# leerob/pixo

Hardware: NVIDIA H100
Metric: Mpixels/sec JPEG q=80 4:2:0 encode of 3840x2160 RGB (higher is better)
Workload: dtype f32

## Files before the change

### pixo_b200/csrc/api.cu

```cuda
#include <stdarg.h>
#include <stdlib.h>
#include <string.h>

#include <emmintrin.h>

#include <algorithm>
#include <cmath>
#include <thread>
#include <vector>

#include "common.cuh"
#include "jpeg_host.hpp"

namespace pixo {

static thread_local std::string g_thread_err;

int set_error(pixo_b200_ctx *ctx, int code, const char *fmt, ...)
{
    char buf[512];
    va_list ap;
    va_start(ap, fmt);
    vsnprintf(buf, sizeof buf, fmt, ap);
    va_end(ap);
// ... 1026 lines not shown
                                         uint32_t n_frames, uint32_t width, uint32_t height, uint32_t color_type,
                                         uint32_t subsampling, const uint8_t *dht, uint8_t *d_out,
                                         size_t out_cap_each, uint64_t *d_scan_len, uint32_t *d_overflow)
{
    if (!ctx) return set_error(nullptr, PIXO_B200_ERR_INVALID_ARGUMENT, "ctx is null");
    PIXO_TRY(validate_jpeg(ctx, width, height, color_type, subsampling));
    const bool chroma = color_type != PIXO_B200_GRAY;
    if (!d_y || !d_out || !d_scan_len || !d_overflow || (chroma && (!d_cb || !d_cr)))
        return set_error(ctx, PIXO_B200_ERR_INVALID_ARGUMENT, "null buffer");
    const FrameGeometry g = make_geometry(width, height, color_type, subsampling);
    auto mis = [](const int16_t *p) { return (reinterpret_cast<uintptr_t>(p) & 15) != 0; };
    if (mis(d_y) || (chroma && (mis(d_cb) || mis(d_cr))))
        return set_error(ctx, PIXO_B200_ERR_INVALID_ARGUMENT, "coefficient arrays must be 16-byte aligned");
    if ((y_stride & 7) || (chroma && (c_stride & 7)))
        return set_error(ctx, PIXO_B200_ERR_INVALID_ARGUMENT, "coefficient strides must be multiples of 8 elements");
    if (n_frames > 1 && (y_stride < g.ny * 64 || (chroma && c_stride < g.nc * 64)))
        return set_error(ctx, PIXO_B200_ERR_INVALID_ARGUMENT,
                         "coefficient strides must hold a frame's blocks (%zu / %zu elements)", g.ny * 64, g.nc * 64);
    ProgTables T;
    {
        HuffTables std_t;
        uint8_t bits[4][16];
        const uint8_t *vals[4];
        if (dht) {
            for (int k = 0; k < 4; ++k) {
                memcpy(bits[k], dht + k * 272, 16);
                vals[k] = dht + k * 272 + 16;
            }
        } else {
            huff_standard(std_t);
            for (int k = 0; k < 4; ++k) {
                memcpy(bits[k], std_t.bits[k], 16);
                vals[k] = std_t.vals[k];
            }
        }
        if (!prog_tables(bits, vals, &T))
            return set_error(ctx, PIXO_B200_ERR_INVALID_ARGUMENT,
                             "Huffman table: more than 256 values, or a code that does not fit its length");
    }
    if (n_frames == 0) return 0;
    PIXO_CUDA(ctx, cudaSetDevice(ctx->device));
    constexpr uint32_t kPass = 8192;
    const int16_t *cb = chroma ? d_cb : nullptr, *cr = chroma ? d_cr : nullptr;
    auto at = [](const int16_t *a, size_t stride, uint32_t i0) { return a ? a + (size_t)i0 * stride : nullptr; };
    ProgResult res;
    if (n_frames > kPass)
        for (uint32_t i0 = 0; i0 < n_frames; i0 += kPass)
            PIXO_TRY(launch_progressive(ctx, at(d_y, y_stride, i0), y_stride, at(cb, c_stride, i0), at(cr, c_stride, i0),
                                        c_stride, std::min(kPass, n_frames - i0), g, &T, false, true, &res));
    for (uint32_t i0 = 0; i0 < n_frames; i0 += kPass) {
        const uint32_t cnt = std::min(kPass, n_frames - i0);
        PIXO_TRY(launch_progressive(ctx, at(d_y, y_stride, i0), y_stride, at(cb, c_stride, i0), at(cr, c_stride, i0),
                                    c_stride, cnt, g, &T, false, false, &res));
        PIXO_TRY(launch_progressive_pack(ctx, res, cnt, d_out + (size_t)i0 * out_cap_each, out_cap_each,
                                         d_scan_len + (size_t)i0 * 7, d_overflow + i0));
    }
    return 0;
}

int pixo_b200_jpeg_encode_dev(pixo_b200_ctx *ctx, const uint8_t *d_pixels, size_t pixel_stride,
                              uint32_t n_images, uint32_t width, uint32_t height,
                              uint32_t color_type, uint32_t quality, uint32_t subsampling,
                              uint8_t *d_scan, size_t scan_cap_each, uint64_t *d_scan_len,
                              uint32_t *d_overflow)
{
    if (!ctx) return set_error(nullptr, PIXO_B200_ERR_INVALID_ARGUMENT, "ctx is null");
    PIXO_TRY(validate_options(ctx, quality, 0));
    PIXO_TRY(validate_jpeg(ctx, width, height, color_type, subsampling));
    if (!d_pixels || !d_scan || !d_scan_len || !d_overflow)
        return set_error(ctx, PIXO_B200_ERR_INVALID_ARGUMENT, "null buffer");
    if (n_images == 0) return 0;
    if (n_images > 65535) return set_error(ctx, PIXO_B200_ERR_INVALID_ARGUMENT, "at most 65535 frames per call");
    if (scan_cap_each % 4 || (reinterpret_cast<uintptr_t>(d_scan) & 15))
        return set_error(ctx, PIXO_B200_ERR_INVALID_ARGUMENT, "scan buffer must be 16-byte aligned, capacity multiple of 4");
    const FrameGeometry g = make_geometry(width, height, color_type, subsampling);
    float lum[64], chr[64];
    quant_tables((int)quality, nullptr, nullptr, lum, chr);
    const CoefLayout L(g);
    PIXO_CUDA(ctx, cudaSetDevice(ctx->device));
    PIXO_TRY(ensure_dev(ctx, ctx->d_coef, (size_t)n_images * L.each));
    PIXO_TRY(ensure_dev(ctx, ctx->d_ent, entropy_scratch_bytes(n_images, g, 0)));
    void *c = ctx->d_coef.ptr;
    const CoefExtents ec = L.extents(c);
    PIXO_TRY(launch_jpeg_transform(ctx, d_pixels, pixel_stride, n_images, width, height, color_type, subsampling,
                                   lum, chr, L.y(c), L.stride(), g.has_chroma ? L.cb(c) : nullptr,
                                   g.has_chroma ? L.cr(c) : nullptr, L.stride(), 0, &ec));
    HuffTables t;
    huff_standard(t);
    uint64_t *len_src = nullptr;
    uint32_t *ovf_src = nullptr;
    PIXO_TRY(launch_jpeg_entropy(ctx, L.y(c), L.stride(), L.cb(c), L.cr(c), L.stride(), n_images, g, t, 0, true, &ec,
                                 reinterpret_cast<uint8_t *>(ctx->d_ent.ptr), d_scan, scan_cap_each,
                                 &len_src, &ovf_src));
    PIXO_CUDA(ctx, cudaMemcpyAsync(d_scan_len, len_src, (size_t)n_images * 8, cudaMemcpyDeviceToDevice, ctx->stream));
    PIXO_CUDA(ctx, cudaMemcpyAsync(d_overflow, ovf_src, (size_t)n_images * 4, cudaMemcpyDeviceToDevice, ctx->stream));
    return 0;
}

static int check_range(pixo_b200_ctx *ctx, const int16_t *y, const int16_t *cb, const int16_t *cr,
                       const FrameGeometry &g, uint32_t restart_interval, const int32_t *seed)
{
    if (!coefficients_in_range(y, g.ny, restart_interval, g.y_per_mcu, seed ? seed[0] : 0) ||
        (g.has_chroma && (!coefficients_in_range(cb, g.nc, restart_interval, 1, seed ? seed[1] : 0) ||
                          !coefficients_in_range(cr, g.nc, restart_interval, 1, seed ? seed[2] : 0))))
        return set_error(ctx, PIXO_B200_ERR_INVALID_ARGUMENT, "%s", kOutOfRange);
    return 0;
}

static int check_coef_alignment(pixo_b200_ctx *ctx, const int16_t *d_y, const int16_t *d_cb, const int16_t *d_cr,
                                bool has_chroma)
{
    auto mis = [](const int16_t *p) { return (reinterpret_cast<uintptr_t>(p) & 15) != 0; };
    if (mis(d_y) || (has_chroma && (mis(d_cb) || mis(d_cr))))
        return set_error(ctx, PIXO_B200_ERR_INVALID_ARGUMENT, "coefficient arrays must be 16-byte aligned");
    return 0;
}

int pixo_b200_jpeg_entropy_encode(pixo_b200_ctx *ctx, const int16_t *y, const int16_t *cb,
                                  const int16_t *cr, uint32_t width, uint32_t height,
                                  uint32_t color_type, uint32_t quality, uint32_t subsampling,
                                  uint32_t restart_interval, uint32_t optimize_huffman,
                                  uint8_t *out, size_t out_cap, size_t *out_len)
{
    PIXO_TRY(validate_options(ctx, quality, restart_interval));
    PIXO_TRY(validate_jpeg(ctx, width, height, color_type, subsampling));
    if (!y || !out || !out_len || (color_type != PIXO_B200_GRAY && (!cb || !cr)))
        return set_error(ctx, PIXO_B200_ERR_INVALID_ARGUMENT, "null buffer");
    const FrameGeometry g = make_geometry(width, height, color_type, subsampling);
    PIXO_TRY(check_range(ctx, y, cb, cr, g, restart_interval, nullptr));
    if (out_cap < 1024 + 2)
        return set_error(ctx, PIXO_B200_ERR_OUTPUT_TOO_SMALL, "output capacity %zu too small", out_cap);
    uint64_t hist[536];
    if (optimize_huffman) host_histogram(y, cb, cr, g, restart_interval, hist);
    HuffTables t;
    tables_from(optimize_huffman ? hist : nullptr, g.has_chroma, t);
    uint8_t lum_zz[64], chr_zz[64];
    quant_tables((int)quality, lum_zz, chr_zz, nullptr, nullptr);
    const size_t hdr = write_headers(out, g, lum_zz, chr_zz, t, restart_interval);
    int threads = ctx ? ctx->host_threads : (int)std::thread::hardware_concurrency();
    const size_t body = entropy_encode_scan(y, cb, cr, g, t, restart_interval, false, out + hdr, out_cap - hdr - 2,
                                            threads < 1 ? 1 : threads);
    return finish_frame(ctx, out, out_cap, hdr, body, out_len);
}

int pixo_b200_jpeg_entropy_encode_dev(pixo_b200_ctx *ctx, const int16_t *d_y, const int16_t *d_cb,
                                      const int16_t *d_cr, uint32_t width, uint32_t height,
                                      uint32_t color_type, uint32_t quality, uint32_t subsampling,
                                      uint32_t restart_interval, uint32_t optimize_huffman,
                                      uint8_t *out, size_t out_cap, size_t *out_len)
{
    if (!ctx) return set_error(nullptr, PIXO_B200_ERR_INVALID_ARGUMENT, "ctx is null");
    PIXO_TRY(validate_options(ctx, quality, restart_interval));
    PIXO_TRY(validate_jpeg(ctx, width, height, color_type, subsampling));
    if (!d_y || !out || !out_len || (color_type != PIXO_B200_GRAY && (!d_cb || !d_cr)))
        return set_error(ctx, PIXO_B200_ERR_INVALID_ARGUMENT, "null buffer");
    if (out_cap < 1024 + 2)
        return set_error(ctx, PIXO_B200_ERR_OUTPUT_TOO_SMALL, "output capacity %zu too small", out_cap);
    const FrameGeometry g = make_geometry(width, height, color_type, subsampling);
    PIXO_TRY(check_coef_alignment(ctx, d_y, d_cb, d_cr, g.has_chroma));
    uint8_t lum_zz[64], chr_zz[64];
    quant_tables((int)quality, lum_zz, chr_zz, nullptr, nullptr);
    PIXO_CUDA(ctx, cudaSetDevice(ctx->device));
    uint64_t *h_hist = nullptr;
    if (optimize_huffman) {
        PIXO_TRY(ensure_dev(ctx, ctx->d_misc, kHistWords * sizeof(uint64_t) + 256));
        PIXO_TRY(ensure_pinned(ctx, ctx->h_misc, kHistWords * sizeof(uint64_t) + 256));
        auto *d_hist = reinterpret_cast<uint64_t *>(ctx->d_misc.ptr);
        h_hist = reinterpret_cast<uint64_t *>(ctx->h_misc.ptr);
        PIXO_TRY(launch_jpeg_histogram(ctx, d_y, 0, d_cb, d_cr, 0, 1, g.ny, g.nc, g.y_per_mcu, restart_interval,
                                       false, nullptr, d_hist));
        PIXO_CUDA(ctx, cudaMemcpyAsync(h_hist, d_hist, kHistWords * sizeof(uint64_t), cudaMemcpyDeviceToHost, ctx->stream));
        PIXO_CUDA(ctx, cudaStreamSynchronize(ctx->stream));
    }
    HuffTables t;
    tables_from(h_hist, g.has_chroma, t);
    const size_t hdr = write_headers(out, g, lum_zz, chr_zz, t, restart_interval);
    const size_t raw = (size_t)width * height * (color_type == PIXO_B200_GRAY ? 1 : 3);
// ... 458 lines not shown
```

### pixo_b200/csrc/common.cuh

```cuda
#pragma once

#include <cuda_runtime.h>
#include <stdint.h>
#include <stdio.h>

#include <atomic>
#include <condition_variable>
#include <functional>
#include <mutex>
#include <string>
#include <thread>
#include <unordered_map>
#include <vector>

#include "../../include/pixo_b200.h"

namespace pixo {

constexpr int kHistWords = 536;

__host__ __device__ constexpr int zz_nat(int i)
{
    constexpr int t[64] = {0,  1,  8,  16, 9,  2,  3,  10, 17, 24, 32, 25, 18, 11, 4,  5,
                           12, 19, 26, 33, 40, 48, 41, 34, 27, 20, 13, 6,  7,  14, 21, 28,
// ... 63 lines not shown
    size_t stage_cap = 0;
    uint64_t *d_len = nullptr;
    std::vector<uint64_t> len;
};

}

struct pixo_b200_ctx {
    int device = 0;
    cudaStream_t own_stream = nullptr;
    cudaStream_t stream = nullptr;
    cudaStream_t copy_stream = nullptr;
    cudaStream_t d2h_stream = nullptr;
    int sm_count = 0;
    int host_threads = 0;
    uint64_t launches = 0;
    uint64_t host_fallbacks = 0;
    size_t scan_cap_override = 0;
    bool gpu_retry = true;
    std::string err;
    pixo::Scratch d_in, d_y, d_cb, d_cr, d_misc, d_out, d_ent, d_coef, d_retry, d_raw;
    pixo::Scratch d_red, d_red_idx, d_red_img;
    pixo::Scratch d_quant, d_quant_img;
    pixo::Scratch d_trellis, h_trellis;
    pixo::Scratch d_prog, d_prog_raw, d_prog_out, h_prog;
    pixo::Scratch h_in, h_out, h_misc, h_red, h_quant;
    std::vector<cudaEvent_t> events;
    std::vector<cudaEvent_t> stage_events;
    pixo::HostPool *pool = nullptr;
    std::unordered_map<const void *, pixo::SegPlan> bands;
};

namespace pixo {

int set_error(pixo_b200_ctx *ctx, int code, const char *fmt, ...);
int cuda_fail(pixo_b200_ctx *ctx, cudaError_t e, const char *what);
int ensure_dev(pixo_b200_ctx *ctx, Scratch &s, size_t bytes);
int ensure_pinned(pixo_b200_ctx *ctx, Scratch &s, size_t bytes);

#define PIXO_CUDA(ctx, call)                                            \
    do {                                                                \
        cudaError_t e__ = (call);                                       \
        if (e__ != cudaSuccess) return ::pixo::cuda_fail(ctx, e__, #call); \
    } while (0)

#define PIXO_TRY(expr)                 \
    do {                               \
        int rc__ = (expr);             \
        if (rc__ != 0) return rc__;    \
    } while (0)

int launch_jpeg_transform(pixo_b200_ctx *ctx, const uint8_t *d_pixels, size_t pixel_stride,
                          uint32_t n_images, uint32_t w, uint32_t h, uint32_t color_type,
                          uint32_t subsampling, const float *lum_q, const float *chr_q,
                          int16_t *d_y, size_t y_stride, int16_t *d_cb, int16_t *d_cr,
                          size_t c_stride, uint32_t flags, const CoefExtents *ext = nullptr);
int launch_jpeg_transform_dct(pixo_b200_ctx *ctx, const uint8_t *d_pixels, size_t pixel_stride, uint32_t n_images,
                              uint32_t w, uint32_t h, uint32_t color_type, uint32_t subsampling,
                              const float *lum_q, const float *chr_q, float *d_y, size_t y_stride, float *d_cb,
                              float *d_cr, size_t c_stride);
int launch_trellis(pixo_b200_ctx *ctx, const float *d_src, size_t src_stride, int16_t *d_dst, size_t dst_stride,
                   uint64_t nb, uint32_t n_frames, const float q[64], float lambda, bool zigzag, uint32_t *d_status);
int launch_jpeg_histogram(pixo_b200_ctx *ctx, const int16_t *d_y, size_t y_stride,
                          const int16_t *d_cb, const int16_t *d_cr, size_t c_stride,
                          uint32_t n_images, size_t ny, size_t nc, uint32_t blocks_y_per_mcu,
                          uint32_t restart_interval, bool zigzag_in, const CoefExtents *ext, uint64_t *d_hist,
                          const int *dc_seed = nullptr);
int launch_png_filter_rows(pixo_b200_ctx *ctx, const uint8_t *d_data, size_t in_stride, uint32_t n_images,
                           uint32_t width, uint32_t height, size_t row_bytes, uint32_t bpp, uint32_t strategy,
                           uint8_t *d_out, size_t out_stride, uint32_t *d_adler, const uint8_t *d_above,
                           uint32_t rule_height);
int launch_adler32(pixo_b200_ctx *ctx, const uint8_t *d_data, size_t len, uint32_t *d_out);
int png_reduce_filter(pixo_b200_ctx *ctx, const uint8_t *d_data, size_t in_stride, uint32_t n_images,
                      uint32_t width, uint32_t height, uint32_t color_type, uint32_t strategy_and_flags,
                      pixo_b200_png_reduced *info, uint8_t *d_out, size_t out_stride, uint32_t *d_adler);
int png_quantize_filter(pixo_b200_ctx *ctx, const uint8_t *d_data, size_t in_stride, uint32_t n_images,
                        uint32_t width, uint32_t height, uint32_t color_type, uint32_t strategy_and_flags,
                        uint32_t max_colors, const uint8_t *palettes, const uint32_t *palette_lens,
                        pixo_b200_png_reduced *info, uint8_t *d_out, size_t out_stride, uint32_t *d_adler);

struct FrameGeometry;
struct HuffTables;
size_t entropy_scratch_bytes(uint32_t n, const FrameGeometry &g, uint32_t restart_interval);
int launch_jpeg_entropy(pixo_b200_ctx *ctx, const int16_t *d_y, size_t y_stride, const int16_t *d_cb,
                        const int16_t *d_cr, size_t c_stride, uint32_t n, const FrameGeometry &g,
                        const HuffTables &t, uint32_t restart_interval, bool allow_segments,
                        const CoefExtents *ext, uint8_t *d_scratch, uint8_t *d_out, uint64_t out_cap,
                        uint64_t **d_out_len, uint32_t **d_overflow);
int launch_band_entropy(pixo_b200_ctx *ctx, const int16_t *d_y, const int16_t *d_cb, const int16_t *d_cr,
                        const FrameGeometry &g, const HuffTables &t, const int dc_seed[3], const int *d_dc_seed,
                        bool allow_segments, uint8_t *d_raw, uint64_t raw_cap, uint64_t *d_bits_tail,
                        uint32_t *d_flags);
int launch_band_splice(pixo_b200_ctx *ctx, const uint8_t *d_raw, uint64_t base_bit, uint32_t base_tail, bool last,
                       const uint64_t *d_base, uint8_t *d_out, uint64_t out_cap, uint64_t *d_out_len,
                       uint32_t *d_flags);
size_t band_raw_bytes(const FrameGeometry &g);
SegPlan splice_plan(uint32_t n, size_t raw_cap);
int launch_splice(pixo_b200_ctx *ctx, uint32_t n, const SegPlan &sp, uint8_t *seg_scratch, const uint8_t *raw_area,
                  uint8_t *d_out, uint64_t out_cap, uint64_t *d_out_len, uint32_t *d_overflow);

bool prog_tables(const uint8_t bits[4][16], const uint8_t *const vals[4], ProgTables *T);
ProgLayout prog_layout(const FrameGeometry &g, uint32_t n);
int launch_progressive(pixo_b200_ctx *ctx, const int16_t *d_y, size_t y_stride, const int16_t *d_cb,
                       const int16_t *d_cr, size_t c_stride, uint32_t n, const FrameGeometry &g,
                       const ProgTables *T, bool per_frame, bool check_only, ProgResult *res);
int launch_progressive_pack(pixo_b200_ctx *ctx, const ProgResult &res, uint32_t n, uint8_t *d_out, uint64_t out_cap,
                            uint64_t *d_scan_len, uint32_t *d_overflow);

}
```

### pixo_b200/csrc/jpeg_entropy.cu

```cuda
#include "common.cuh"
#include "jpeg_host.hpp"

namespace pixo {
namespace {

constexpr int AC_STRIDE = 12, AC_ZRL = 190, AC_EOB = 191, AC_WORDS = 192;
struct HuffDev {
    uint32_t dc[2][12];
    uint32_t ac[2][AC_WORDS];
};

struct EntParams {
    const int16_t *y, *cb, *cr;
    size_t y_stride, c_stride;
    CoefExtents e;
    uint32_t bpm;
    uint32_t y_per_mcu;
    uint32_t nblocks;
    uint32_t nchunks;
    uint32_t rst_mcus;
    uint32_t rst_blocks;
    uint32_t cpi;
    uint32_t nimages;
    unsigned long long *st_bits;
// ... 185 lines not shown
        while (mb) {
            const uint32_t f = msb_index(mb);
            uint32_t bit;
            asm("bmsk.clamp.b32 %0, %1, 1;" : "=r"(bit) : "r"(f));
            mb ^= bit;
            const uint32_t pos = top - f;
            uint32_t run = pos + nprev;
            nprev = ~pos;
            uint32_t caddr;
            asm("{\n\t.reg .b32 h, x;\n\tand.b32 h, %1, 1;\n\tmad.lo.u32 x, %1, 64, %2;\n\tmad.lo.u32 %0, h, -62, x;\n\t}"
                : "=r"(caddr) : "r"(pos), "r"(sa_stage));
            const int c = lds_s16(caddr);
#pragma unroll 1
            while (run >= 16u) { put(zrl & 0xFFFF0000u, zrl & 31u); run -= 16u; }
            const uint32_t a = (uint32_t)abs(c);
            if (CHECK) amax |= a >> 10;
            const uint32_t lz = CHECK ? max((uint32_t)__clz((int)a), 22u) : (uint32_t)__clz((int)a);
            const uint32_t e = lds_u32(sa_ac_top + run * (AC_STRIDE * 4u) - lz * 4u);
            const uint32_t amp = a ^ ((uint32_t)(c >> 31) >> lz);
            const uint32_t n = e & 31u;
            put((e & 0xFFFF0000u) | __funnelshift_r(0u, amp, n), n);
        }
    }
    if (nprev != ~63u) put(eob & 0xFFFF0000u, eob & 31u);
    *acc_out = acc;
    *bad = amax != 0;
    return ((sp - sa_slot) / (CB * 4)) * 32u + filled;
}

__device__ __forceinline__ uint32_t warp_scan(uint32_t x, int lane, uint32_t *total)
{
    uint32_t inc = x;
#pragma unroll
    for (int o = 1; o < 32; o <<= 1) {
        const uint32_t n = __shfl_up_sync(0xffffffffu, inc, o);
        if (lane >= o) inc += n;
    }
    *total = __shfl_sync(0xffffffffu, inc, 31);
    return inc - x;
}

struct WarpMem {
    uint32_t slot[2][SLOT_W * CB];
    union {
        uint32_t stage[32 * CB];
        struct {
            uint32_t obuf[WIN_W];
            uint8_t sbuf[SBUF_B];
        } w;
    };
    uint32_t tl[CB];
};

struct ChunkState {
    uint32_t chunk, img;
    uint32_t L, o_t;
    int nwt;
    uint32_t Lc, ctail;
    int buf;
    unsigned long long Pc;
    uint32_t tailin;
    uint32_t Ftot;
    uint32_t own;
    uint32_t marker;
    bool first, last, final_;
    uint32_t ffb;
    bool kept;
    bool fault;
    bool skip;
};

template <bool RAW, bool CHECK>
__global__ void __launch_bounds__(32 * HUFF_WARPS, HUFF_CTAS_PER_SM)
k_huff(const __grid_constant__ EntParams P, const __grid_constant__ HuffDev Tp)
{
    __shared__ HuffDev T;
    __shared__ __align__(16) WarpMem wmem[HUFF_WARPS];
    static_assert(sizeof(((WarpMem *)0)->w) <= sizeof(((WarpMem *)0)->stage), "window + stuffed bytes must fit the stage");

    const int lane = threadIdx.x & 31;
    for (int i = threadIdx.x; i < (int)(sizeof(HuffDev) / 4); i += blockDim.x)
        reinterpret_cast<uint32_t *>(&T)[i] = reinterpret_cast<const uint32_t *>(&Tp)[i];
    __syncthreads();
    WarpMem &M = wmem[threadIdx.x >> 5];
    uint32_t *const obuf = M.w.obuf;
    uint8_t *const sbuf = M.w.sbuf;
    const uint32_t sa_stage = (uint32_t)__cvta_generic_to_shared(M.stage) + 4u * lane;
    const uint32_t total_chunks = P.nchunks * P.nimages;
    uint32_t spill[2][MAX_W - SLOT_W];

    auto phase_w = [&](uint32_t id, int buf, ChunkState &C) {
        C.chunk = id / P.nimages;
        C.img = id - C.chunk * P.nimages;
        C.buf = buf;
        C.fault = false;
        uint32_t s0, iend, interval = 0;
        uint32_t nblk = P.nblocks;
        size_t y_off = (size_t)C.img * P.y_stride, c_off = (size_t)C.img * P.c_stride;
        size_t ey_off = (size_t)C.img * P.e.stride, ec_off = ey_off;
        bool seg_prev = false;
        if (RAW && P.seg_per_img > 1) {
            const uint32_t ii = C.img / P.seg_per_img, seg = C.img - ii * P.seg_per_img;
            y_off = (size_t)ii * P.y_stride + (size_t)seg * P.seg_y_stride;
            c_off = (size_t)ii * P.c_stride + (size_t)seg * P.seg_c_stride;
            ey_off = (size_t)ii * P.e.stride + (size_t)seg * (P.seg_y_stride / 64);
            ec_off = (size_t)ii * P.e.stride + (size_t)seg * (P.seg_c_stride / 64);
            if (seg == P.seg_per_img - 1) nblk = P.nblocks_last;
            seg_prev = seg != 0;
        }
        C.skip = false;
        if (P.rst_blocks) {
            interval = C.chunk / P.cpi;
            const uint32_t sub = C.chunk - interval * P.cpi;
            s0 = interval * P.rst_blocks + sub * CB;
            iend = (uint32_t)min((unsigned long long)(interval + 1) * P.rst_blocks, (unsigned long long)nblk);
            C.first = sub == 0;
        } else {
            s0 = C.chunk * CB;
            iend = nblk;
            C.first = C.chunk == 0;
        }
        if (s0 >= iend) { C.skip = true; return; }
        C.last = s0 + CB >= iend;
        C.final_ = C.last && iend == nblk;
        C.marker = (C.last && !C.final_) ? 0xD0u + (interval & 7u) : 0u;
        const uint32_t s = s0 + lane;
        const int nv = (int)min((uint32_t)CB, iend - s0);
        uint32_t *const slot = M.slot[buf];
        uint32_t L = 0, tail7 = 0;
        int nwt = 0;
        uint32_t M0 = 0, M1 = 0;
        int diff = 0, tbl = 0;
        if (s < iend) {
            const uint32_t m = s / P.bpm;
            const uint32_t k = s - m * P.bpm;
            const int16_t *arr;
            const uint8_t *earr;
            size_t idx, eidx;
            int seed;
            if (k < P.y_per_mcu) { arr = P.y + y_off; earr = P.e.y; idx = (size_t)m * P.y_per_mcu + k; eidx = ey_off + idx; tbl = 0; seed = P.dc_seed[0]; }
            else if (k == P.y_per_mcu) { arr = P.cb + c_off; earr = P.e.cb; idx = m; eidx = ec_off + idx; tbl = 1; seed = P.dc_seed[1]; }
            else { arr = P.cr + c_off; earr = P.e.cr; idx = m; eidx = ec_off + idx; tbl = 1; seed = P.dc_seed[2]; }
            const bool dc_reset = P.rst_mcus && m % P.rst_mcus == 0 && (k == 0 || k >= P.y_per_mcu);
            if (P.dc_seed_dev && idx == 0 && !seg_prev) seed = P.dc_seed_dev[k < P.y_per_mcu ? 0 : (k == P.y_per_mcu ? 1 : 2)];
            const int prev_dc = dc_reset ? 0 : ((idx || seg_prev) ? arr[((long long)idx - 1) * 64] : seed);
            const uint4 *src = reinterpret_cast<const uint4 *>(arr + idx * 64);
            int dc;
            uint32_t w[32];
            if (CHECK) {
                uint32_t n[32];
#pragma unroll
                for (int q = 0; q < 8; ++q) {
                    const uint4 v = __ldg(src + q);
                    n[q * 4] = v.x; n[q * 4 + 1] = v.y; n[q * 4 + 2] = v.z; n[q * 4 + 3] = v.w;
                }
                dc = (int)(int16_t)(n[0] & 0xFFFF);
#pragma unroll
                for (int j = 0; j < 32; ++j) {
                    const int i0 = zz_nat(2 * j), i1 = zz_nat(2 * j + 1);
                    w[j] = __byte_perm(n[i0 >> 1], n[i1 >> 1],
                                       ((i0 & 1) ? 0x0032 : 0x0010) | ((i1 & 1) ? 0x7600 : 0x5400));
                }
#pragma unroll
                for (int j = 0; j < 32; ++j) M.stage[j * CB + lane] = w[j];
            } else {
                const int np = 2 * __ldg(earr + eidx);
// ... 714 lines not shown

static SegPlan plan_segments(uint32_t n, uint32_t S, uint64_t total_mcus, uint64_t bpm, uint64_t mcu_raw_bytes)
{
    SegPlan p;
    p.seg_mcus = (total_mcus + S - 1) / S;
    S = (uint32_t)((total_mcus + p.seg_mcus - 1) / p.seg_mcus);
    p.S = S;
    p.last_mcus = total_mcus - p.seg_mcus * (S - 1);
    const uint64_t fair = p.seg_mcus * mcu_raw_bytes + 4096, worst = p.seg_mcus * bpm * 216 + 64;
    lay_out(p, n, bpm, (size_t)a256(std::min(fair, worst)));
    return p;
}

static uint64_t mcu_raw_bytes(const FrameGeometry &g) { return (uint64_t)g.y_per_mcu * 64 * (g.has_chroma ? 3 : 1); }

static int code_segments(pixo_b200_ctx *ctx, EntParams P, const HuffDev &T, uint32_t n, const FrameGeometry &g,
                         const SegPlan &sp, uint8_t *seg_scratch, uint8_t *raw_area)
{
    const bool check = P.e.y == nullptr;
    cudaStream_t st = ctx->stream;
    const uint64_t bpm = g.y_per_mcu + (g.has_chroma ? 2 : 0);
    uint8_t *ent = seg_scratch + sp.off_ent;
    P.nimages = n * sp.S;
    P.seg_per_img = sp.S;
    P.nblocks = (uint32_t)(sp.seg_mcus * bpm);
    P.nblocks_last = (uint32_t)(sp.last_mcus * bpm);
    P.nchunks = (uint32_t)sp.ent.nchunks;
    P.seg_y_stride = (size_t)sp.seg_mcus * g.y_per_mcu * 64;
    P.seg_c_stride = (size_t)sp.seg_mcus * 64;
    P.rst_blocks = P.rst_mcus = P.cpi = 0;
    P.st_bits = reinterpret_cast<unsigned long long *>(ent + sp.ent.off_st1);
    P.st_ff = reinterpret_cast<unsigned long long *>(ent + sp.ent.off_st2);
    P.ticket = reinterpret_cast<uint32_t *>(ent + sp.ent.off_ticket);
    P.overflow = reinterpret_cast<uint32_t *>(ent + sp.ent.off_ovf);
    P.out_len = reinterpret_cast<uint64_t *>(ent + sp.ent.off_outlen);
    P.out_tail = reinterpret_cast<unsigned long long *>(ent + sp.ent.off_tail);
    P.out = raw_area;
    P.out_cap = sp.raw_cap;
    PIXO_CUDA(ctx, cudaMemsetAsync(ent, 0, sp.ent.zero_bytes, st));
    const size_t want = ((size_t)P.nimages * P.nchunks + HUFF_WARPS - 1) / HUFF_WARPS;
    const unsigned grid = (unsigned)std::min<size_t>(want, (size_t)ctx->sm_count * HUFF_CTAS_PER_SM);
    if (check) k_huff<true, true><<<grid, 32 * HUFF_WARPS, 0, st>>>(P, T);
    else k_huff<true, false><<<grid, 32 * HUFF_WARPS, 0, st>>>(P, T);
    ctx->launches += 1;
    PIXO_CUDA(ctx, cudaGetLastError());
    PIXO_CUDA(ctx, cudaMemcpyAsync(raw_area + sp.off_bits, P.out_len, (size_t)n * sp.S * 8, cudaMemcpyDeviceToDevice, st));
    PIXO_CUDA(ctx, cudaMemcpyAsync(raw_area + sp.off_tails, P.out_tail, (size_t)n * sp.S * 8, cudaMemcpyDeviceToDevice, st));
    return 0;
}

static int splice_segments(pixo_b200_ctx *ctx, uint32_t n, const SegPlan &sp, uint8_t *seg_scratch,
                           const uint8_t *raw_area, const uint32_t *raw_overflow, uint64_t base_bit, uint32_t base_tail,
                           bool last, const uint64_t *base_dev, uint8_t *d_out, uint64_t out_cap, uint64_t *d_out_len,
                           uint32_t *d_overflow)
{
    cudaStream_t st = ctx->stream;
    SegParams Q;
    Q.raw = raw_area; Q.raw_cap = sp.raw_cap;
    Q.bits = reinterpret_cast<const unsigned long long *>(raw_area + sp.off_bits);
    Q.tails = reinterpret_cast<const unsigned long long *>(raw_area + sp.off_tails);
    Q.S = sp.S; Q.max_tiles = sp.max_tiles;
    Q.base_bit = base_bit; Q.base_tail = base_tail; Q.last_band = last ? 1u : 0u;
    Q.base_dev = reinterpret_cast<const unsigned long long *>(base_dev);
    Q.rec = reinterpret_cast<SegRec *>(seg_scratch + sp.off_rec);
    Q.ntiles = reinterpret_cast<uint32_t *>(seg_scratch + sp.off_ntiles);
    Q.cnt = reinterpret_cast<uint32_t *>(seg_scratch + sp.off_cnt);
    Q.out = d_out; Q.out_cap = out_cap;
    Q.out_len = reinterpret_cast<unsigned long long *>(d_out_len);
    Q.overflow = d_overflow;
    Q.raw_overflow = raw_overflow;
    k_seg_prefix<<<n, SPL_THREADS, 0, st>>>(Q);
    k_seg_count<<<dim3((sp.max_tiles + SPL_TPC - 1) / SPL_TPC, n), SPL_THREADS, 0, st>>>(Q);
    k_seg_scan<<<n, 1024, 0, st>>>(Q);
    k_seg_emit<<<dim3((sp.max_tiles + SPL_TPC - 1) / SPL_TPC, n), SPL_THREADS, 0, st>>>(Q);
    ctx->launches += 4;
    PIXO_CUDA(ctx, cudaGetLastError());
    return 0;
}

int launch_jpeg_entropy(pixo_b200_ctx *ctx, const int16_t *d_y, size_t y_stride, const int16_t *d_cb,
                        const int16_t *d_cr, size_t c_stride, uint32_t n, const FrameGeometry &g,
                        const HuffTables &t, uint32_t restart_interval, bool allow_segments,
                        const CoefExtents *ext, uint8_t *d_scratch, uint8_t *d_out, uint64_t out_cap,
                        uint64_t **d_out_len, uint32_t **d_overflow)
{
    const bool check = ext == nullptr;
    const uint64_t nblocks = g.ny + 2 * g.nc;
    const uint64_t bpm_ = g.y_per_mcu + (g.has_chroma ? 2 : 0);
    uint64_t rst_blocks = (uint64_t)restart_interval * bpm_;
    if (rst_blocks >= nblocks) rst_blocks = 0;
    const EntropyPlan pl = plan_entropy(n, nblocks, rst_blocks);
    if (nblocks > 0xFFFFFFFFull || (uint64_t)n * pl.nchunks > 0x7FFFFFFFull)
        return set_error(ctx, PIXO_B200_ERR_INVALID_ARGUMENT, "entropy stage: too many blocks per call");
    EntParams P;
    P.y = d_y; P.cb = d_cb; P.cr = d_cr; P.y_stride = y_stride; P.c_stride = c_stride;
    P.e = ext ? *ext : CoefExtents{nullptr, nullptr, nullptr, 0};
    P.bpm = g.y_per_mcu + (g.has_chroma ? 2 : 0);
    P.y_per_mcu = g.y_per_mcu;
    P.nblocks = (uint32_t)nblocks;
    P.nchunks = (uint32_t)pl.nchunks;
    P.rst_blocks = (uint32_t)rst_blocks;
    P.rst_mcus = rst_blocks ? restart_interval : 0u;
    P.cpi = rst_blocks ? (uint32_t)((rst_blocks + CB - 1) / CB) : 0u;
    P.nimages = n;
    P.st_bits = reinterpret_cast<unsigned long long *>(d_scratch + pl.off_st1);
    P.st_ff = reinterpret_cast<unsigned long long *>(d_scratch + pl.off_st2);
    P.ticket = reinterpret_cast<uint32_t *>(d_scratch + pl.off_ticket);
    P.overflow = reinterpret_cast<uint32_t *>(d_scratch + pl.off_ovf);
    P.out_len = reinterpret_cast<uint64_t *>(d_scratch + pl.off_outlen);
    P.out = d_out; P.out_cap = out_cap;
    P.out_tail = reinterpret_cast<unsigned long long *>(d_scratch + pl.off_tail);
    P.dc_seed[0] = P.dc_seed[1] = P.dc_seed[2] = 0;
    P.dc_seed_dev = nullptr;
    *d_out_len = P.out_len;
    *d_overflow = P.overflow;

    HuffDev T;
    make_huff_dev(t, &T);
    cudaStream_t st = ctx->stream;
    PIXO_CUDA(ctx, cudaMemsetAsync(d_scratch, 0, pl.zero_bytes, st));
    P.seg_per_img = 1; P.nblocks_last = P.nblocks; P.seg_y_stride = P.seg_c_stride = 0;
    const uint32_t S = (rst_blocks == 0 && allow_segments) ? segments_for(n, g.total_mcus(), bpm_) : 1;
    const SegPlan sp = plan_segments(n, S, g.total_mcus(), bpm_, mcu_raw_bytes(g));
    if (sp.S > 1) {
        PIXO_TRY(ensure_dev(ctx, ctx->d_raw, sp.total + sp.raw_total));
        auto *seg_scratch = reinterpret_cast<uint8_t *>(ctx->d_raw.ptr);
        uint8_t *raw_area = seg_scratch + sp.total;
        PIXO_TRY(code_segments(ctx, P, T, n, g, sp, seg_scratch, raw_area));
        return splice_segments(ctx, n, sp, seg_scratch, raw_area,
                               reinterpret_cast<const uint32_t *>(seg_scratch + sp.off_ent + sp.ent.off_ovf), 0, 0, true,
                               nullptr, d_out, out_cap, P.out_len, P.overflow);
    }
    const size_t want = ((size_t)n * pl.nchunks + HUFF_WARPS - 1) / HUFF_WARPS;
    const unsigned grid = (unsigned)std::min<size_t>(want, (size_t)ctx->sm_count * HUFF_CTAS_PER_SM);
    if (check) k_huff<false, true><<<grid, 32 * HUFF_WARPS, 0, st>>>(P, T);
    else k_huff<false, false><<<grid, 32 * HUFF_WARPS, 0, st>>>(P, T);
    ctx->launches += 1;
    PIXO_CUDA(ctx, cudaGetLastError());
    return 0;
}

size_t band_raw_bytes(const FrameGeometry &g)
{
    return plan_segments(1, 1, g.total_mcus(), g.y_per_mcu + (g.has_chroma ? 2 : 0), mcu_raw_bytes(g)).raw_total;
}

int launch_band_entropy(pixo_b200_ctx *ctx, const int16_t *d_y, const int16_t *d_cb, const int16_t *d_cr,
                        const FrameGeometry &g, const HuffTables &t, const int dc_seed[3], const int *d_dc_seed,
                        bool allow_segments, uint8_t *d_raw, uint64_t raw_cap, uint64_t *d_bits_tail,
                        uint32_t *d_flags)
{
    if ((g.ny + 2 * g.nc) > 0xFFFFFFFFull)
        return set_error(ctx, PIXO_B200_ERR_INVALID_ARGUMENT, "entropy stage: too many blocks per call");
    const uint64_t bpm = g.y_per_mcu + (g.has_chroma ? 2 : 0);
    SegPlan sp = plan_segments(1, allow_segments ? segments_for(1, g.total_mcus(), bpm) : 1, g.total_mcus(), bpm,
                               mcu_raw_bytes(g));
    if (sp.S == 1 || sp.raw_total > raw_cap) {
        sp = plan_segments(1, 1, g.total_mcus(), bpm, mcu_raw_bytes(g));
        const size_t trailer = sp.raw_total - sp.raw_bytes;
        if (raw_cap < trailer)
            return set_error(ctx, PIXO_B200_ERR_OUTPUT_TOO_SMALL, "raw capacity %llu too small (need %zu)",
                             (unsigned long long)raw_cap, sp.raw_total);
        lay_out(sp, 1, bpm, (size_t)(raw_cap - trailer) / 256 * 256);
    }
    PIXO_TRY(ensure_dev(ctx, ctx->d_raw, sp.total));
    auto *seg_scratch = reinterpret_cast<uint8_t *>(ctx->d_raw.ptr);
    EntParams P;
    memset(&P, 0, sizeof P);
    P.y = d_y; P.cb = d_cb; P.cr = d_cr;
    P.bpm = (uint32_t)bpm; P.y_per_mcu = g.y_per_mcu;
    for (int k = 0; k < 3; ++k) P.dc_seed[k] = dc_seed ? dc_seed[k] : 0;
    P.dc_seed_dev = d_dc_seed;
    HuffDev T;
    make_huff_dev(t, &T);
    ctx->bands[d_raw] = sp;
    PIXO_TRY(code_segments(ctx, P, T, 1, g, sp, seg_scratch, d_raw));
    k_band_totals<<<1, 32, 0, ctx->stream>>>(reinterpret_cast<const unsigned long long *>(d_raw + sp.off_bits),
                                             reinterpret_cast<const unsigned long long *>(d_raw + sp.off_tails),
                                             reinterpret_cast<const uint32_t *>(seg_scratch + sp.off_ent + sp.ent.off_ovf), sp.S,
                                             reinterpret_cast<unsigned long long *>(d_bits_tail), d_flags);
    ctx->launches += 1;
    PIXO_CUDA(ctx, cudaGetLastError());
    return 0;
}

int launch_band_splice(pixo_b200_ctx *ctx, const uint8_t *d_raw, uint64_t base_bit, uint32_t base_tail, bool last,
                       const uint64_t *d_base, uint8_t *d_out, uint64_t out_cap, uint64_t *d_out_len,
                       uint32_t *d_flags)
{
    const auto it = ctx->bands.find(d_raw);
    if (it == ctx->bands.end())
        return set_error(ctx, PIXO_B200_ERR_INVALID_ARGUMENT, "this raw buffer was not coded by pixo_b200_jpeg_band_entropy_dev");
    const SegPlan sp = it->second;
    PIXO_TRY(ensure_dev(ctx, ctx->d_raw, sp.total));
    return splice_segments(ctx, 1, sp, reinterpret_cast<uint8_t *>(ctx->d_raw.ptr), d_raw, nullptr, base_bit, base_tail,
                           last, d_base, d_out, out_cap, d_out_len, d_flags);
}

SegPlan splice_plan(uint32_t n, size_t raw_cap)
{
    SegPlan p;
    p.S = 1;
    p.seg_mcus = p.last_mcus = 0;
    lay_out(p, n, 1, raw_cap);
    return p;
}

int launch_splice(pixo_b200_ctx *ctx, uint32_t n, const SegPlan &sp, uint8_t *seg_scratch, const uint8_t *raw_area,
                  uint8_t *d_out, uint64_t out_cap, uint64_t *d_out_len, uint32_t *d_overflow)
{
    return splice_segments(ctx, n, sp, seg_scratch, raw_area, nullptr, 0, 0, true, nullptr, d_out, out_cap, d_out_len,
                           d_overflow);
}

}
```

### pixo_b200/csrc/jpeg_transform.cu

```cuda
#include <cuda.h>
#include <string.h>

#include <algorithm>

#include "common.cuh"

namespace pixo {
namespace {

#define FADD(a, b) __fadd_rn((a), (b))
#define FSUB(a, b) __fsub_rn((a), (b))
#define FMUL(a, b) __fmul_rn((a), (b))

#define AAN_A1 0.70710678118654752440f
#define AAN_A2 0.5411961f
#define AAN_A3 0.70710678118654752440f
#define AAN_A4 1.3065629f
#define AAN_A5 0.38268343f
#define AAN_S0 0.3535534f
#define AAN_S1 0.2548978f
#define AAN_S2 0.2705981f
#define AAN_S3 0.3006724f
#define AAN_S4 0.3535534f
#define AAN_S5 0.4499881f
// ... 365 lines not shown
constexpr int K1_MIN_BLOCKS = 2;
constexpr int K1_MCUS = 16;
constexpr int K1_HB = 8 * 16 * 3;
constexpr int K1_HALF_BYTES = 16 * K1_HB;
constexpr int K1_TILE_BYTES = 2 * K1_HALF_BYTES;

struct K1Params {
    const uint8_t *pixels;
    size_t pixel_stride;
    uint32_t w, h, mcus_x, mcus_y, units_x, n_images;
    int16_t *y, *cb, *cr;
    size_t y_stride, c_stride;
    CoefExtents e;
    uint32_t use_tma;
};

struct __align__(128) K1WarpSmem {
    uint8_t tile[2][K1_HALF_BYTES];
    uint32_t csum[K1_MCUS * 64];
    __align__(16) uint8_t ext[32];
    uint64_t bar;
};

struct __align__(128) K1Smem {
    K1WarpSmem w[K1_WARPS];
    QPairTab q;
};

__device__ __forceinline__ void rgb_windows8(const uint32_t (&w)[6], uint32_t (&win)[8])
{
    win[0] = w[0];
    win[1] = __funnelshift_r(w[0], w[1], 24);
    win[2] = __funnelshift_r(w[1], w[2], 16);
    win[3] = w[2] >> 8;
    win[4] = w[3];
    win[5] = __funnelshift_r(w[3], w[4], 24);
    win[6] = __funnelshift_r(w[4], w[5], 16);
    win[7] = w[5] >> 8;
}

__device__ __forceinline__ void ycc_row8(const uint32_t (&w)[6], float (&yv)[8], uint32_t (&hs)[4])
{
    uint32_t win[8];
    rgb_windows8(w, win);
    uint32_t pp[8];
#pragma unroll
    for (int x = 0; x < 8; ++x) {
        const uint32_t ys = __dp4a(win[x], 0x001D964Du, 128u);
        const int ucb = dp4a_us(win[x], 0x0080552Bu, -32641);
        const int ucr = dp4a_us(win[x], 0x00156B80u, -32641);
        yv[x] = __uint_as_float(__byte_perm(ys, 0x4B000000u, 0x7651));
        pp[x] = __vmaxu2(__byte_perm((uint32_t)ucb, (uint32_t)ucr, 0x7531), 0xFF01FF01u);
    }
#pragma unroll
    for (int k = 0; k < 4; ++k) hs[k] = pp[2 * k] + pp[2 * k + 1];
}

template <int ROWS, int TILE_PX>
__device__ __noinline__ void warp_load_tile_rgb(uint8_t *__restrict__ smem,
                                                   const uint8_t *__restrict__ img, uint32_t w,
                                                   uint32_t h, uint32_t x0, uint32_t y0, int lane)
{
    load_tile<3, ROWS, TILE_PX, 32>(smem, img, w, h, x0, y0, lane);
}

template <int OUT>
__global__ void __launch_bounds__(K1_THREADS, K1_MIN_BLOCKS)
k_jpeg_420(const __grid_constant__ K1Params P, const __grid_constant__ QPairTab qp,
           const __grid_constant__ CUtensorMap tmap)
{
    extern __shared__ __align__(128) uint8_t smem_raw[];
    K1Smem &S = *reinterpret_cast<K1Smem *>(smem_raw);
    const int tid = threadIdx.x;
    const int lane = tid & 31, warp = tid >> 5;
    K1WarpSmem &WS = S.w[warp];
    for (int i = tid; i < 64; i += K1_THREADS) S.q.t[i >> 5][i & 31] = qp.t[i >> 5][i & 31];
    const QPairTab *QS = &S.q;

    if (lane == 0) {
        mbar_init(&WS.bar, 1);
        asm volatile("fence.mbarrier_init.release.cluster;" ::: "memory");
    }
    __syncthreads();

    const uint32_t units_per_img = P.mcus_y * P.units_x;
    const uint64_t nunits = (uint64_t)units_per_img * P.n_images;
    const uint32_t stride = gridDim.x * K1_WARPS;
    const uint32_t d_ux = stride % P.units_x, d_t = stride / P.units_x;
    const uint32_t d_my = d_t % P.mcus_y, d_img = d_t / P.mcus_y;
    uint32_t phase = 0;

    auto advance = [&](uint32_t &img, uint32_t &my, uint32_t &ux) {
        ux += d_ux;
        if (ux >= P.units_x) { ux -= P.units_x; ++my; }
        my += d_my;
        if (my >= P.mcus_y) { my -= P.mcus_y; ++img; }
        img += d_img;
    };
    auto unit_by_tma = [&](uint32_t my) { return P.use_tma && (my * 16 + 16 <= P.h); };
    auto issue_tma = [&](uint32_t img_, uint32_t my_, uint32_t ux_) {
        if (unit_by_tma(my_)) {
            asm volatile("fence.proxy.async.shared::cta;" ::: "memory");
            mbar_expect_tx(&WS.bar, K1_TILE_BYTES);
            tma_load_3d(WS.tile[0], &tmap, (int)(ux_ * (2 * K1_HB / 8)), (int)(my_ * 16), (int)img_, &WS.bar);
            tma_load_3d(WS.tile[1], &tmap, (int)(ux_ * (2 * K1_HB / 8) + K1_HB / 8), (int)(my_ * 16), (int)img_, &WS.bar);
        }
    };
    auto load_half = [&](uint32_t img_, uint32_t my_, uint32_t ux_, int half) {
        const uint8_t *image = P.pixels + (size_t)img_ * P.pixel_stride;
        const uint32_t x0 = ux_ * (K1_MCUS * 16) + half * 128;
        if (x0 < P.w) warp_load_tile_rgb<16, 128>(WS.tile[half], image, P.w, P.h, x0, my_ * 16, lane);
        __syncwarp();
    };

    uint64_t u = (uint64_t)blockIdx.x * K1_WARPS + warp;
    uint32_t img, my, ux;
    {
        const uint32_t u0 = blockIdx.x * K1_WARPS + warp;
        img = u0 / units_per_img;
        const uint32_t rem = u0 - img * units_per_img;
        my = rem / P.units_x;
        ux = rem - my * P.units_x;
    }
    if (u < nunits && lane == 0) issue_tma(img, my, ux);

    for (; u < nunits; u += stride) {
        if (unit_by_tma(my)) {
            mbar_wait(&WS.bar, phase);
            phase ^= 1;
        } else {
            load_half(img, my, ux, 0);
            load_half(img, my, ux, 1);
        }
        uint32_t img_n = img, my_n = my, ux_n = ux;
        advance(img_n, my_n, ux_n);
        const uint32_t mcu0 = ux * K1_MCUS;
        const uint32_t n_mcu = min((uint32_t)K1_MCUS, P.mcus_x - mcu0);
        const size_t mcu_base = (size_t)my * P.mcus_x + mcu0;

#pragma unroll 1
        for (int job = 0; job < 3; ++job) {
            const bool chroma_u = __ballot_sync(0xffffffffu, job == 2) != 0u;
            f2 R[4][8];
            uint4 *stage;
            int slot, swz;
            if (!chroma_u) {
                const int by = lane >> 4, l16 = lane & 15;
                const int par = l16 >> 3, k8 = l16 & 7;
                const int mj = (k8 >> 1) * 2 + par;
                const int mcu = job * 8 + mj;
                const int bx = k8 & 1;
                const uint8_t *base = WS.tile[job] + (by * 8) * K1_HB + (mj * 2 + bx) * 24;
                uint4 *cdst = reinterpret_cast<uint4 *>(WS.csum) + mcu * 16;
#pragma unroll
                for (int rp = 0; rp < 4; ++rp) {
                    float y0[8], y1[8];
                    uint32_t h0[4], h1[4];
                    {
                        const uint2 *p = reinterpret_cast<const uint2 *>(base + (rp * 2) * K1_HB);
                        const uint2 a = p[0], b = p[1], c = p[2];
                        const uint32_t wds[6] = {a.x, a.y, b.x, b.y, c.x, c.y};
                        ycc_row8(wds, y0, h0);
                    }
                    {
                        const uint2 *p = reinterpret_cast<const uint2 *>(base + (rp * 2 + 1) * K1_HB);
                        const uint2 a = p[0], b = p[1], c = p[2];
// ... 60 lines not shown
                uint4 *ybase = reinterpret_cast<uint4 *>(P.y + (size_t)img * P.y_stride + b0 * 64);
                const uint32_t first = job * 8;
                flush_stage<OUT>(
                    stage, WS.ext, lane, [](int s) { return ((s >> 3) << 1) | (s & 1); },
                    [&](int s) -> uint4 * { return first + (s >> 2) < n_mcu ? ybase + s * 8 : nullptr; },
                    [&](int s) -> uint8_t * {
                        return first + (s >> 2) < n_mcu ? P.e.y + ((size_t)img * P.e.stride + b0 + s) : nullptr;
                    });
            } else {
                uint4 *cbb = reinterpret_cast<uint4 *>(P.cb + (size_t)img * P.c_stride + mcu_base * 64);
                uint4 *crb = reinterpret_cast<uint4 *>(P.cr + (size_t)img * P.c_stride + mcu_base * 64);
                flush_stage<OUT>(
                    stage, WS.ext, lane, [](int s) { return s & 7; },
                    [&](int s) -> uint4 * {
                        return (uint32_t)(s & 15) < n_mcu ? (s < 16 ? cbb : crb) + (s & 15) * 8 : nullptr;
                    },
                    [&](int s) -> uint8_t * {
                        return (uint32_t)(s & 15) < n_mcu
                                   ? (s < 16 ? P.e.cb : P.e.cr) + ((size_t)img * P.e.stride + mcu_base + (s & 15))
                                   : nullptr;
                    });
            }
        }
        img = img_n; my = my_n; ux = ux_n;
    }
}

constexpr int GRAY_BLOCKS = 64;

__device__ __forceinline__ void y_row8(const uint32_t (&w)[6], float (&v)[8])
{
    uint32_t win[8];
    rgb_windows8(w, win);
#pragma unroll
    for (int x = 0; x < 8; ++x)
        v[x] = byte1_to_float_minus(__dp4a(win[x], 0x001D964Du, 128u), 8388736.0f);
}
__device__ __forceinline__ void c_row8(const uint32_t (&w)[6], uint32_t wgt, float (&v)[8])
{
    uint32_t win[8];
    rgb_windows8(w, win);
#pragma unroll
    for (int x = 0; x < 8; ++x) {
        const int u = max(dp4a_us(win[x], wgt, -32641), -65280);
        v[x] = FSUB(8388736.0f, __uint_as_float(__byte_perm((uint32_t)u, 0x4B000000u, 0x7651)));
    }
}

constexpr int K444_WARPS = 4;
constexpr int K444_THREADS = K444_WARPS * 32;
constexpr int K444_ROW_B = 32 * 8 * 3;
constexpr int K444_TILE_BYTES = 8 * K444_ROW_B;
constexpr int K444_MIN_BLOCKS = 2;

struct __align__(128) K444WarpSmem {
    uint8_t tile[2][K444_TILE_BYTES];
    uint4 stage[256];
    __align__(16) uint8_t ext[32];
    uint64_t bar[2];
};

struct __align__(128) K444Smem {
    K444WarpSmem w[K444_WARPS];
    QPairTab q;
};

template <int OUT>
__global__ void __launch_bounds__(K444_THREADS, K444_MIN_BLOCKS)
k_jpeg_444(const __grid_constant__ K1Params P, const __grid_constant__ QPairTab qp,
           const __grid_constant__ CUtensorMap tmap)
{
    extern __shared__ __align__(128) uint8_t smem_raw[];
    K444Smem &S = *reinterpret_cast<K444Smem *>(smem_raw);
    const int tid = threadIdx.x, lane = tid & 31, warp = tid >> 5;
    K444WarpSmem &WS = S.w[warp];
    for (int i = tid; i < 64; i += K444_THREADS) S.q.t[i >> 5][i & 31] = qp.t[i >> 5][i & 31];
    const QPairTab *QS = &S.q;
    if (lane == 0) {
        mbar_init(&WS.bar[0], 1);
        mbar_init(&WS.bar[1], 1);
        asm volatile("fence.mbarrier_init.release.cluster;" ::: "memory");
    }
    __syncthreads();

    const uint32_t units_per_img = P.mcus_y * P.units_x;
    const uint64_t nunits = (uint64_t)units_per_img * P.n_images;
    const uint32_t stride = gridDim.x * K444_WARPS;
    const uint32_t d_ux = stride % P.units_x, d_t = stride / P.units_x;
    const uint32_t d_by = d_t % P.mcus_y, d_img = d_t / P.mcus_y;
    uint32_t phase = 0;

    auto advance = [&](uint32_t &img, uint32_t &by, uint32_t &ux) {
        ux += d_ux;
        if (ux >= P.units_x) { ux -= P.units_x; ++by; }
        by += d_by;
        if (by >= P.mcus_y) { by -= P.mcus_y; ++img; }
        img += d_img;
    };
    auto unit_by_tma = [&](uint32_t by) { return P.use_tma && (by * 8 + 8 <= P.h); };
    auto issue_tma = [&](uint32_t img_, uint32_t by_, uint32_t ux_, int b) {
        if (unit_by_tma(by_)) {
            asm volatile("fence.proxy.async.shared::cta;" ::: "memory");
            mbar_expect_tx(&WS.bar[b], K444_TILE_BYTES);
            tma_load_3d(WS.tile[b], &tmap, (int)(ux_ * (K444_ROW_B / 8)), (int)(by_ * 8), (int)img_, &WS.bar[b]);
        }
    };

    uint64_t u = (uint64_t)blockIdx.x * K444_WARPS + warp;
    uint32_t img, by, ux;
    {
        const uint32_t u0 = blockIdx.x * K444_WARPS + warp;
        img = u0 / units_per_img;
        const uint32_t rem = u0 - img * units_per_img;
        by = rem / P.units_x;
        ux = rem - by * P.units_x;
    }
    int b = 0;
    if (u < nunits && lane == 0) issue_tma(img, by, ux, 0);
    for (; u < nunits; u += stride, b ^= 1) {
        uint32_t img_n = img, by_n = by, ux_n = ux;
        advance(img_n, by_n, ux_n);
        if (lane == 0 && u + stride < nunits) issue_tma(img_n, by_n, ux_n, b ^ 1);
        if (unit_by_tma(by)) {
            mbar_wait(&WS.bar[b], (phase >> b) & 1u);
            phase ^= 1u << b;
        } else {
            const uint8_t *image = P.pixels + (size_t)img * P.pixel_stride;
            warp_load_tile_rgb<8, 256>(WS.tile[b], image, P.w, P.h, ux * 256, by * 8, lane);
            __syncwarp();
        }
        const uint32_t bx0 = ux * 32;
        const uint8_t *base = WS.tile[b] + lane * 24;
        auto row_words = [&](int r, uint32_t (&wds)[6]) {
            const uint2 *p = reinterpret_cast<const uint2 *>(base + r * K444_ROW_B);
            const uint2 a = p[0], c1 = p[1], c2 = p[2];
            wds[0] = a.x; wds[1] = a.y; wds[2] = c1.x; wds[3] = c1.y; wds[4] = c2.x; wds[5] = c2.y;
        };
        const size_t b0 = (size_t)by * P.mcus_x + bx0;
        auto flush = [&](int16_t *arr, uint8_t *earr) {
            uint4 *dbase = reinterpret_cast<uint4 *>(arr + b0 * 64);
            flush_stage<OUT>(
                WS.stage, WS.ext, lane, [](int s) { return s & 7; },
                [&](int s) -> uint4 * { return bx0 + s < P.mcus_x ? dbase + s * 8 : nullptr; },
                [&](int s) -> uint8_t * { return bx0 + s < P.mcus_x ? earr + s : nullptr; });
        };
#pragma unroll 1
        for (int comp = 0; comp < 3; ++comp) {
            const bool chroma_u = __ballot_sync(0xffffffffu, comp != 0) != 0u;
            f2 R[4][8];
            if (!chroma_u) {
#pragma unroll
                for (int rp = 0; rp < 4; ++rp) {
                    float v0[8], v1[8];
                    uint32_t wa[6], wb[6];
                    row_words(rp * 2, wa); row_words(rp * 2 + 1, wb);
                    y_row8(wa, v0); y_row8(wb, v1);
#pragma unroll
                    for (int x = 0; x < 8; ++x) R[rp][x] = pk(v0[x], v1[x]);
                }
            } else {
                const uint32_t wgt = comp == 1 ? 0x0080552Bu : 0x00156B80u;
#pragma unroll
                for (int rp = 0; rp < 4; ++rp) {
                    float v0[8], v1[8];
                    uint32_t wa[6], wb[6];
                    row_words(rp * 2, wa); row_words(rp * 2 + 1, wb);
// ... 347 lines not shown
```

Before: 192,700.

## Overlap transform and entropy kernels with programmatic dependent launch

Launches the Huffman entropy kernel with programmatic stream serialization. The transform kernels trigger launch_dependents early and the entropy kernel waits with griddepcontrol.wait after loading its tables, so its launch and prologue can overlap the transform's tail. The scratch memset moves ahead of the transform so it does not sit between the two kernels and break the dependency chain. The entropy kernel also writes lengths straight into the caller's buffer, which removes one device-to-device copy. Early-launched entropy CTAs may hold SM slots while the transform is still running.

Measured after the change: 192,800, median of 6. No clear change (+0.1%).

```diff
diff --git a/pixo_b200/csrc/api.cu b/pixo_b200/csrc/api.cu
--- a/pixo_b200/csrc/api.cu
+++ b/pixo_b200/csrc/api.cu
@@ -1132,6 +1132,8 @@
     PIXO_TRY(ensure_dev(ctx, ctx->d_ent, entropy_scratch_bytes(n_images, g, 0)));
     void *c = ctx->d_coef.ptr;
     const CoefExtents ec = L.extents(c);
+    auto *ent = reinterpret_cast<uint8_t *>(ctx->d_ent.ptr);
+    PIXO_TRY(clear_entropy_scratch(ctx, n_images, g, ent));
     PIXO_TRY(launch_jpeg_transform(ctx, d_pixels, pixel_stride, n_images, width, height, color_type, subsampling,
                                    lum, chr, L.y(c), L.stride(), g.has_chroma ? L.cb(c) : nullptr,
                                    g.has_chroma ? L.cr(c) : nullptr, L.stride(), 0, &ec));
@@ -1139,10 +1141,11 @@
     huff_standard(t);
     uint64_t *len_src = nullptr;
     uint32_t *ovf_src = nullptr;
+    const EntropyFollows follows{d_scan_len};
     PIXO_TRY(launch_jpeg_entropy(ctx, L.y(c), L.stride(), L.cb(c), L.cr(c), L.stride(), n_images, g, t, 0, true, &ec,
-                                 reinterpret_cast<uint8_t *>(ctx->d_ent.ptr), d_scan, scan_cap_each,
-                                 &len_src, &ovf_src));
-    PIXO_CUDA(ctx, cudaMemcpyAsync(d_scan_len, len_src, (size_t)n_images * 8, cudaMemcpyDeviceToDevice, ctx->stream));
+                                 ent, d_scan, scan_cap_each, &len_src, &ovf_src, &follows));
+    if (len_src != d_scan_len)
+        PIXO_CUDA(ctx, cudaMemcpyAsync(d_scan_len, len_src, (size_t)n_images * 8, cudaMemcpyDeviceToDevice, ctx->stream));
     PIXO_CUDA(ctx, cudaMemcpyAsync(d_overflow, ovf_src, (size_t)n_images * 4, cudaMemcpyDeviceToDevice, ctx->stream));
     return 0;
 }
diff --git a/pixo_b200/csrc/common.cuh b/pixo_b200/csrc/common.cuh
--- a/pixo_b200/csrc/common.cuh
+++ b/pixo_b200/csrc/common.cuh
@@ -169,11 +169,15 @@
 struct FrameGeometry;
 struct HuffTables;
 size_t entropy_scratch_bytes(uint32_t n, const FrameGeometry &g, uint32_t restart_interval);
+struct EntropyFollows {
+    uint64_t *out_len;
+};
 int launch_jpeg_entropy(pixo_b200_ctx *ctx, const int16_t *d_y, size_t y_stride, const int16_t *d_cb,
                         const int16_t *d_cr, size_t c_stride, uint32_t n, const FrameGeometry &g,
                         const HuffTables &t, uint32_t restart_interval, bool allow_segments,
                         const CoefExtents *ext, uint8_t *d_scratch, uint8_t *d_out, uint64_t out_cap,
-                        uint64_t **d_out_len, uint32_t **d_overflow);
+                        uint64_t **d_out_len, uint32_t **d_overflow, const EntropyFollows *follows = nullptr);
+int clear_entropy_scratch(pixo_b200_ctx *ctx, uint32_t n, const FrameGeometry &g, uint8_t *d_scratch);
 int launch_band_entropy(pixo_b200_ctx *ctx, const int16_t *d_y, const int16_t *d_cb, const int16_t *d_cr,
                         const FrameGeometry &g, const HuffTables &t, const int dc_seed[3], const int *d_dc_seed,
                         bool allow_segments, uint8_t *d_raw, uint64_t raw_cap, uint64_t *d_bits_tail,
diff --git a/pixo_b200/csrc/jpeg_entropy.cu b/pixo_b200/csrc/jpeg_entropy.cu
--- a/pixo_b200/csrc/jpeg_entropy.cu
+++ b/pixo_b200/csrc/jpeg_entropy.cu
@@ -291,6 +291,7 @@
     for (int i = threadIdx.x; i < (int)(sizeof(HuffDev) / 4); i += blockDim.x)
         reinterpret_cast<uint32_t *>(&T)[i] = reinterpret_cast<const uint32_t *>(&Tp)[i];
     __syncthreads();
+    asm volatile("griddepcontrol.wait;" ::: "memory");
     WarpMem &M = wmem[threadIdx.x >> 5];
     uint32_t *const obuf = M.w.obuf;
     uint8_t *const sbuf = M.w.sbuf;
@@ -1171,7 +1172,7 @@
                         const int16_t *d_cr, size_t c_stride, uint32_t n, const FrameGeometry &g,
                         const HuffTables &t, uint32_t restart_interval, bool allow_segments,
                         const CoefExtents *ext, uint8_t *d_scratch, uint8_t *d_out, uint64_t out_cap,
-                        uint64_t **d_out_len, uint32_t **d_overflow)
+                        uint64_t **d_out_len, uint32_t **d_overflow, const EntropyFollows *follows)
 {
     const bool check = ext == nullptr;
     const uint64_t nblocks = g.ny + 2 * g.nc;
@@ -1207,7 +1208,7 @@
     HuffDev T;
     make_huff_dev(t, &T);
     cudaStream_t st = ctx->stream;
-    PIXO_CUDA(ctx, cudaMemsetAsync(d_scratch, 0, pl.zero_bytes, st));
+    if (!follows) PIXO_CUDA(ctx, cudaMemsetAsync(d_scratch, 0, pl.zero_bytes, st));
     P.seg_per_img = 1; P.nblocks_last = P.nblocks; P.seg_y_stride = P.seg_c_stride = 0;
     const uint32_t S = (rst_blocks == 0 && allow_segments) ? segments_for(n, g.total_mcus(), bpm_) : 1;
     const SegPlan sp = plan_segments(n, S, g.total_mcus(), bpm_, mcu_raw_bytes(g));
@@ -1222,10 +1223,33 @@
     }
     const size_t want = ((size_t)n * pl.nchunks + HUFF_WARPS - 1) / HUFF_WARPS;
     const unsigned grid = (unsigned)std::min<size_t>(want, (size_t)ctx->sm_count * HUFF_CTAS_PER_SM);
-    if (check) k_huff<false, true><<<grid, 32 * HUFF_WARPS, 0, st>>>(P, T);
-    else k_huff<false, false><<<grid, 32 * HUFF_WARPS, 0, st>>>(P, T);
+    if (follows) {
+        if (follows->out_len) *d_out_len = P.out_len = follows->out_len;
+        cudaLaunchAttribute attr;
+        attr.id = cudaLaunchAttributeProgrammaticStreamSerialization;
+        attr.val.programmaticStreamSerializationAllowed = 1;
+        cudaLaunchConfig_t cfg = {};
+        cfg.gridDim = dim3(grid);
+        cfg.blockDim = dim3(32 * HUFF_WARPS);
+        cfg.stream = st;
+        cfg.attrs = &attr;
+        cfg.numAttrs = 1;
+        if (check) PIXO_CUDA(ctx, cudaLaunchKernelEx(&cfg, k_huff<false, true>, P, T));
+        else PIXO_CUDA(ctx, cudaLaunchKernelEx(&cfg, k_huff<false, false>, P, T));
+    } else if (check) {
+        k_huff<false, true><<<grid, 32 * HUFF_WARPS, 0, st>>>(P, T);
+    } else {
+        k_huff<false, false><<<grid, 32 * HUFF_WARPS, 0, st>>>(P, T);
+    }
     ctx->launches += 1;
     PIXO_CUDA(ctx, cudaGetLastError());
+    return 0;
+}
+
+int clear_entropy_scratch(pixo_b200_ctx *ctx, uint32_t n, const FrameGeometry &g, uint8_t *d_scratch)
+{
+    const EntropyPlan pl = plan_entropy(n, g.ny + 2 * g.nc, 0);
+    PIXO_CUDA(ctx, cudaMemsetAsync(d_scratch, 0, pl.zero_bytes, ctx->stream));
     return 0;
 }
 
diff --git a/pixo_b200/csrc/jpeg_transform.cu b/pixo_b200/csrc/jpeg_transform.cu
--- a/pixo_b200/csrc/jpeg_transform.cu
+++ b/pixo_b200/csrc/jpeg_transform.cu
@@ -471,6 +471,7 @@
         asm volatile("fence.mbarrier_init.release.cluster;" ::: "memory");
     }
     __syncthreads();
+    asm volatile("griddepcontrol.launch_dependents;" ::: "memory");
 
     const uint32_t units_per_img = P.mcus_y * P.units_x;
     const uint64_t nunits = (uint64_t)units_per_img * P.n_images;
@@ -697,6 +698,7 @@
         asm volatile("fence.mbarrier_init.release.cluster;" ::: "memory");
     }
     __syncthreads();
+    asm volatile("griddepcontrol.launch_dependents;" ::: "memory");
 
     const uint32_t units_per_img = P.mcus_y * P.units_x;
     const uint64_t nunits = (uint64_t)units_per_img * P.n_images;
```
